# barathanaslan/whisper-ipa

Measured on AMD Instinct MI355X. Metric: audio-seconds/sec transcribed (whisper-small, 30s clips), higher is better.
Workload: dtype bf16

## Files before the change

whisper_ipa_amd/csrc/cross_absorbed.hip:

```cpp
#include <cstdlib>
#include <mutex>
#include <type_traits>

#include "attn_stream.h"
#include "wipa_common.h"

namespace {

constexpr int FT = 32;
constexpr long long XA_RESIDENT_MB_SHARED = 16;
constexpr long long XA_RESIDENT_MB_LONE = -1;
typedef __attribute__((address_space(3))) void* lds_ptr_a;
typedef int v2i32 __attribute__((ext_vector_type(2)));

struct AbsParams {
    const __bf16* qp;
    const __bf16* xa;
    float* part_m;
    float* part_l;
    float* part_o;
    int Tk, n_splits, tiles_per_split, H;
    int resident_groups;
};

constexpr int POLICY_DEFAULT = 0, POLICY_NT = 2;

__device__ __forceinline__ int swz(int row) { return (row & 7) << 1; }

// ... 207 lines not shown
typedef __bf16 bf16x4v __attribute__((ext_vector_type(4)));

template <int D, int NW_>
struct AbsCfg2 {
    static constexpr int NWV = NW_;
    static constexpr int GF = 16;
    static constexpr int ROWB = D * 2;
    static constexpr int SLOT = GF * ROWB;
    static constexpr int SMEM_LOOP = NWV * 2 * SLOT;
    static constexpr int MROW = D + 4;
    static constexpr int SMEM_MERGE = NWV * 16 * MROW * 4 + NWV * 32 * 4;
    static constexpr int SMEM = SMEM_LOOP > SMEM_MERGE ? SMEM_LOOP : SMEM_MERGE;
};

#define WIPA_TR8(X, A, IMM)                                                                                                          \
    asm volatile("ds_read_b64_tr_b16 %0, %8 offset:" #IMM "\n\tds_read_b64_tr_b16 %1, %9 offset:" #IMM                              \
                 "\n\tds_read_b64_tr_b16 %2, %10 offset:" #IMM "\n\tds_read_b64_tr_b16 %3, %11 offset:" #IMM                          \
                 "\n\tds_read_b64_tr_b16 %4, %12 offset:" #IMM "\n\tds_read_b64_tr_b16 %5, %13 offset:" #IMM                          \
                 "\n\tds_read_b64_tr_b16 %6, %14 offset:" #IMM "\n\tds_read_b64_tr_b16 %7, %15 offset:" #IMM "\n\ts_waitcnt lgkmcnt(0)" \
                 : "=&v"(X[0]), "=&v"(X[1]), "=&v"(X[2]), "=&v"(X[3]), "=&v"(X[4]), "=&v"(X[5]), "=&v"(X[6]), "=&v"(X[7])           \
                 : "v"(A[0]), "v"(A[1]), "v"(A[2]), "v"(A[3]), "v"(A[4]), "v"(A[5]), "v"(A[6]), "v"(A[7])                           \
                 : "memory")

template <int D, int NW_>
__global__ __launch_bounds__(64 * NW_, 1) void cross_absorbed_v2_kernel(AbsParams p) {
    typedef AbsCfg2<D, NW_> X;
    constexpr int NWV = X::NWV, GF = X::GF, ROWB = X::ROWB, SLOT = X::SLOT;
    constexpr int NDMA = SLOT / 1024;
    constexpr int KS = D / 32;
    constexpr int CT = D / 16;
    static_assert(SLOT % 1024 == 0 && NDMA <= 32 && CT % 8 == 0 && KS % 4 == 0 && CT / 8 <= 8 && D % 128 == 0, "width");
    extern __shared__ __attribute__((aligned(1024))) char smem[];
    const int tid = threadIdx.x, lane = tid & 63;
    const int wave = __builtin_amdgcn_readfirstlane(tid >> 6);
    const int l15 = lane & 15, g = lane >> 4;
    const int split = blockIdx.x, b = blockIdx.y;
    const int groups_total = (p.Tk + GF - 1) / GF;
    const int gps = 2 * p.tiles_per_split;
    const int g0 = split * gps;
    const int ng = max(0, min(gps, groups_total - g0));
    const int my_n = ng > wave ? (ng - wave + NWV - 1) / NWV : 0;
    const __bf16* xb = p.xa + (int64_t)b * p.Tk * D;
    char* my = smem + wave * (2 * SLOT);

    bf16x8 qf[KS];
    {
        const __bf16* qr = p.qp + ((int64_t)b * 16 + l15) * D + 8 * g;
// ... 60 lines not shown
            else if constexpr (NDMA == 16) asm volatile("s_waitcnt vmcnt(16)" ::: "memory");
            else if constexpr (NDMA == 12) asm volatile("s_waitcnt vmcnt(12)" ::: "memory");
            else asm volatile("s_waitcnt vmcnt(0)" ::: "memory");
        } else {
            asm volatile("s_waitcnt vmcnt(0)" ::: "memory");
        }
    };
    auto scores = [&](int slot, int i_local, float& mx) -> f32x4 {
        f32x4 s4[4] = {f32x4{0.f, 0.f, 0.f, 0.f}, f32x4{0.f, 0.f, 0.f, 0.f}, f32x4{0.f, 0.f, 0.f, 0.f}, f32x4{0.f, 0.f, 0.f, 0.f}};
        const int so = slot * SLOT;
#pragma unroll
        for (int ks = 0; ks < KS; ++ks) {
            const bf16x8 a = *reinterpret_cast<const bf16x8*>(sb[ks & 3] + so + 256 * (ks >> 2));
            s4[ks & 3] = __builtin_amdgcn_mfma_f32_16x16x32_bf16(a, qf[ks], s4[ks & 3], 0, 0, 0);
        }
        f32x4 s = (s4[0] + s4[1]) + (s4[2] + s4[3]);
        const int f0 = (g0 + wave + NWV * i_local) * GF;
        mx = NEG_BIG;
#pragma unroll
        for (int r = 0; r < 4; ++r) {
            if (f0 + 4 * g + r >= p.Tk) s[r] = NEG_BIG;
            mx = fmaxf(mx, s[r]);
        }
        mx = fmaxf(mx, __shfl_xor(mx, 16, 64));
        mx = fmaxf(mx, __shfl_xor(mx, 32, 64));
        return s;
    };
    constexpr float DRIFT = 40.f;
    f32x4 acc[CT];
    float m_ref = NEG_BIG, l_run = 0.f;
    bool exact = false;
    for (;;) {
#pragma unroll
        for (int c = 0; c < CT; ++c) acc[c] = f32x4{0.f, 0.f, 0.f, 0.f};
        l_run = 0.f;
        bool drifted = false;
        if (my_n > 0) stage(0, 0);
        if (my_n > 1) stage(1, 1);
        for (int i = 0; i < my_n; ++i) {
            const int slot = i & 1;
            wait_slot(i + 1 < my_n);
            float mx;
            const f32x4 s = scores(slot, i, mx);
            if (i == 0 && !exact) m_ref = mx;
            if (__builtin_amdgcn_ballot_w64(mx > m_ref + DRIFT) != 0) {
                drifted = true;
                break;
            }
            float ls = 0.f;
            bf16x4v pf;
#pragma unroll
            for (int r = 0; r < 4; ++r) {
                const float e = (s[r] <= NEG_TEST) ? 0.f : __expf(s[r] - m_ref);
                pf[r] = (__bf16)e;
                ls += e;
            }
            ls += __shfl_xor(ls, 16, 64);
            ls += __shfl_xor(ls, 32, 64);
            l_run += ls;
            {
                unsigned tas[8];
#pragma unroll
                for (int cc = 0; cc < 8; ++cc) tas[cc] = ta[cc] + slot * SLOT;
#define WIPA_PV_BLK(BLK, IMM)                                                                                                       \
    if constexpr (CT / 8 > BLK) {                                                                                                   \
        v2i32 x[8];                                                                                                                 \
        WIPA_TR8(x, tas, IMM);                                                                                                      \
        _Pragma("unroll") for (int cc = 0; cc < 8; ++cc) acc[8 * BLK + cc] =                                                       \
            __builtin_amdgcn_mfma_f32_16x16x16bf16_1k(pf, __builtin_bit_cast(bf16x4v, x[cc]), acc[8 * BLK + cc], 0, 0, 0);         \
    }
                WIPA_PV_BLK(0, 0)
                WIPA_PV_BLK(1, 256)
                WIPA_PV_BLK(2, 512)
                WIPA_PV_BLK(3, 768)
                WIPA_PV_BLK(4, 1024)
                WIPA_PV_BLK(5, 1280)
                WIPA_PV_BLK(6, 1536)
                WIPA_PV_BLK(7, 1792)
#undef WIPA_PV_BLK
            }
            asm volatile("" ::: "memory");
            if (i + 2 < my_n) stage(i + 2, slot);
        }
        if (!drifted) break;
        asm volatile("s_waitcnt vmcnt(0)" ::: "memory");
        float mt = NEG_BIG;
// ... 15 lines not shown
    asm volatile("s_waitcnt vmcnt(0)" ::: "memory");
    __syncthreads();
    constexpr int RS = X::MROW;
    float* so = reinterpret_cast<float*>(smem);
    float* sm = so + NWV * 16 * RS;
#pragma unroll
    for (int c = 0; c < CT; ++c)
#pragma unroll
        for (int r = 0; r < 4; ++r) so[(wave * 16 + 4 * g + r) * RS + 16 * c + l15] = acc[c][r];
    if (g == 0) {
        sm[wave * 16 + l15] = m_run;
        sm[NWV * 16 + wave * 16 + l15] = l_run;
    }
    __syncthreads();
    const int64_t ps = (int64_t)b * p.n_splits + split;
    float* po = p.part_o + ps * 16 * D;
    for (int hd = 0; hd < p.H; ++hd) {
        float mv[NWV], M = NEG_BIG;
#pragma unroll
        for (int v = 0; v < NWV; ++v) {
            mv[v] = sm[v * 16 + hd];
            M = fmaxf(M, mv[v]);
        }
        for (int c4 = tid; 4 * c4 < D; c4 += NWV * 64) {
            f32x4 o = {0.f, 0.f, 0.f, 0.f};
#pragma unroll
            for (int v = 0; v < NWV; ++v)
                o += __expf(mv[v] - M) * *reinterpret_cast<const f32x4*>(so + (v * 16 + hd) * RS + 4 * c4);
            *reinterpret_cast<f32x4*>(po + hd * D + 4 * c4) = o;
        }
    }
    if (tid < 16) {
        float M = NEG_BIG, Lsum = 0.f;
#pragma unroll
        for (int v = 0; v < NWV; ++v) M = fmaxf(M, sm[v * 16 + tid]);
#pragma unroll
        for (int v = 0; v < NWV; ++v) Lsum += __expf(sm[v * 16 + tid] - M) * sm[NWV * 16 + v * 16 + tid];
        p.part_m[ps * 16 + tid] = M;
        p.part_l[ps * 16 + tid] = Lsum;
    }
}
#undef WIPA_TR8

template <int D>
__global__ __launch_bounds__(64) void cross_absorb_q_kernel(const __bf16* __restrict__ q, int64_t q_rs, const __bf16* __restrict__ wkT,
                                                            __bf16* __restrict__ qp, int B, int H, float scale) {
    constexpr int CT = D / 4 / 16;
    const int lane = threadIdx.x & 63, wave = blockIdx.z;
    const int l15 = lane & 15, g = lane >> 4;
    const int h = blockIdx.x, b0 = blockIdx.y * 16;
    if (h >= H) {
        for (int e = lane; e < 16 * (D / 4); e += 64) {
            const int bb = b0 + e / (D / 4);
            if (bb < B) qp[((int64_t)bb * 16 + h) * D + wave * (D / 4) + e % (D / 4)] = (__bf16)0.f;
        }
        return;
    }
    const int bq = min(b0 + l15, B - 1);
    bf16x8 qa[2];
#pragma unroll
    for (int ks = 0; ks < 2; ++ks) qa[ks] = *reinterpret_cast<const bf16x8*>(q + (int64_t)bq * q_rs + h * 64 + 32 * ks + 8 * g);
    bf16x8 wb[CT][2];
#pragma unroll
    for (int i = 0; i < CT; ++i)
#pragma unroll
// ... 7 lines not shown
        for (int ks = 0; ks < 2; ++ks) acc = __builtin_amdgcn_mfma_f32_16x16x32_bf16(qa[ks], wb[i][ks], acc, 0, 0, 0);
#pragma unroll
        for (int r = 0; r < 4; ++r) {
            const int bb = b0 + 4 * g + r;
            if (bb < B) qp[((int64_t)bb * 16 + h) * D + c0 + l15] = (__bf16)(acc[r] * scale);
        }
    }
}

template <int D>
struct MergeCfg {
#ifndef WIPA_MERGE_KQ
#define WIPA_MERGE_KQ 96
#endif
#ifndef WIPA_MERGE_CL
#define WIPA_MERGE_CL 4
#endif
    static constexpr int KQ = (D % 96 == 0) ? WIPA_MERGE_KQ : (D == 512 ? 64 : 128);
    static constexpr int NWM = D / KQ;
    static constexpr int KS = KQ / 32;
    static constexpr int CL = WIPA_MERGE_CL;
};

template <int D, bool OUTP = false>
__global__ __launch_bounds__(64 * MergeCfg<D>::NWM) void cross_merge_proj_kernel(
    const float* __restrict__ part_m, const float* __restrict__ part_l, const float* __restrict__ part_o, int n_splits,
    const __bf16* __restrict__ wv, const float* __restrict__ bv, __bf16* __restrict__ out, int64_t o_rs, int B,
    const __bf16* __restrict__ wo = nullptr, const float* __restrict__ bo = nullptr, float* __restrict__ slabs_out = nullptr,
    int64_t slab_stride = 0) {
    constexpr int KQ = MergeCfg<D>::KQ, KS = MergeCfg<D>::KS, NWM = MergeCfg<D>::NWM;
    static_assert(KQ % 32 == 0 && NWM * KQ == D, "width");
    constexpr int CL = MergeCfg<D>::CL;
    constexpr int NTO = D / 16;
    constexpr int NTOW = (NTO + NWM - 1) / NWM;
    __shared__ __attribute__((aligned(16))) float red[NWM][CL][64 + 4];
    __shared__ __attribute__((aligned(16))) __bf16 vh[OUTP ? CL : 1][64 + 8];
    const int tid = threadIdx.x, lane = tid & 63, w = tid >> 6;
    const int l15 = lane & 15, g = lane >> 4;
    const int h = blockIdx.x, b0 = blockIdx.y * CL;
    const int bc = min(b0 + (l15 & (CL - 1)), B - 1);
    bf16x8 wq[4][KS];
#pragma unroll
    for (int nt = 0; nt < 4; ++nt)
#pragma unroll
        for (int ks = 0; ks < KS; ++ks)
            wq[nt][ks] = *reinterpret_cast<const bf16x8*>(wv + (int64_t)(h * 64 + 16 * nt + l15) * D + w * KQ + 32 * ks + 8 * g);
    bf16x8 wof[OUTP ? NTOW : 1][2];
    if constexpr (OUTP) {
#pragma unroll
        for (int i = 0; i < NTOW; ++i) {
            const int nt = min(w * NTOW + i, NTO - 1);
#pragma unroll
            for (int ks = 0; ks < 2; ++ks)
                wof[i][ks] = *reinterpret_cast<const bf16x8*>(wo + (int64_t)(16 * nt + l15) * D + h * 64 + 32 * ks + 8 * g);
        }
    }
    float pm[4], pl[4];
#pragma unroll
    for (int s = 0; s < 4; ++s) {
        const int sc = min(s, n_splits - 1);
        pm[s] = part_m[((int64_t)bc * n_splits + sc) * 16 + h];
        pl[s] = part_l[((int64_t)bc * n_splits + sc) * 16 + h];
    }
    f32x4 po[KS][4][2];
#pragma unroll
    for (int ks = 0; ks < KS; ++ks)
#pragma unroll
        for (int s = 0; s < 4; ++s) {
            const int sc = min(s, n_splits - 1);
            const float* pr = part_o + (((int64_t)bc * n_splits + sc) * 16 + h) * D + w * KQ + 32 * ks + 8 * g;
            po[ks][s][0] = *reinterpret_cast<const f32x4*>(pr);
            po[ks][s][1] = *reinterpret_cast<const f32x4*>(pr + 4);
        }
    __builtin_amdgcn_sched_barrier(0);
    float ws[4];
    {
        float M = NEG_BIG;
#pragma unroll
        for (int s = 0; s < 4; ++s)
            if (s < n_splits) M = fmaxf(M, pm[s]);
        float Lsum = 0.f;
#pragma unroll
        for (int s = 0; s < 4; ++s) {
            ws[s] = s < n_splits ? __expf(pm[s] - M) : 0.f;
            Lsum += ws[s] * pl[s];
        }
        const float inv = 1.0f / Lsum;
#pragma unroll
        for (int s = 0; s < 4; ++s) ws[s] *= inv;
    }
    f32x4 acc[4] = {f32x4{0.f, 0.f, 0.f, 0.f}, f32x4{0.f, 0.f, 0.f, 0.f}, f32x4{0.f, 0.f, 0.f, 0.f}, f32x4{0.f, 0.f, 0.f, 0.f}};
#pragma unroll
    for (int ks = 0; ks < KS; ++ks) {
        f32x4 lo = {0.f, 0.f, 0.f, 0.f}, hi = {0.f, 0.f, 0.f, 0.f};
#pragma unroll
        for (int s = 0; s < 4; ++s) {
            lo += ws[s] * po[ks][s][0];
            hi += ws[s] * po[ks][s][1];
        }
        bf16x8 a;
#pragma unroll
        for (int e = 0; e < 4; ++e) {
            a[e] = (__bf16)lo[e];
            a[4 + e] = (__bf16)hi[e];
        }
#pragma unroll
        for (int nt = 0; nt < 4; ++nt) acc[nt] = __builtin_amdgcn_mfma_f32_16x16x32_bf16(a, wq[nt][ks], acc[nt], 0, 0, 0);
    }
    if (4 * g < CL) {
#pragma unroll
        for (int nt = 0; nt < 4; ++nt)
#pragma unroll
            for (int r = 0; r < 4; ++r)
                if (4 * g + r < CL) red[w][4 * g + r][16 * nt + l15] = acc[nt][r];
    }
    __syncthreads();
    for (int e = tid; e < CL * 64; e += 64 * NWM) {
        const int row = e >> 6, j = e & 63;
        float o = 0.f;
#pragma unroll
        for (int v = 0; v < NWM; ++v) o += red[v][row][j];
// ... 156 lines not shown
        for (int e = tid; e < (16 - CG) * 64; e += 512) qh[CG + (e >> 6)][e & 63] = (__bf16)0.f;
    }
    __syncthreads();
    {
        const bf16x8 a0 = *reinterpret_cast<const bf16x8*>(&qh[l15][8 * g]);
        const bf16x8 a1 = *reinterpret_cast<const bf16x8*>(&qh[l15][32 + 8 * g]);
#pragma unroll
        for (int i = 0; i < NTW; ++i) {
            const int nt = wave * NTW + i;
            if (nt < NT) {
                f32x4 acc = {0.f, 0.f, 0.f, 0.f};
                acc = __builtin_amdgcn_mfma_f32_16x16x32_bf16(a0, wkf[i][0], acc, 0, 0, 0);
                acc = __builtin_amdgcn_mfma_f32_16x16x32_bf16(a1, wkf[i][1], acc, 0, 0, 0);
#pragma unroll
                for (int r = 0; r < 4; ++r) {
                    const int bb_ = b0 + 4 * g + r;
                    if (4 * g + r < CG && bb_ < p.B) p.qp[((int64_t)bb_ * 16 + h) * D + 16 * nt + l15] = (__bf16)(acc[r] * p.k_scale);
                }
            }
        }
    }
}

template <int D>
int launch_attn(const AbsParams& p_in, int B, hipStream_t s) {
    const char* e = getenv("WIPA_ABS_KERNEL");
    AbsParams p = p_in;
    p.resident_groups = wipa_cross_absorbed_resident_groups(B, D, p.Tk, p.n_splits);
    if ((e && atoi(e) == 1) || (D > 768 && !(e && atoi(e) == 2)))
        hipLaunchKernelGGL((cross_absorbed_kernel<D>), dim3(p.n_splits, B), dim3(64 * AbsCfg<D>::NW), AbsCfg<D>::SMEM, s, p);
    else if constexpr (D > 768)
        hipLaunchKernelGGL((cross_absorbed_v2_kernel<D, 2>), dim3(p.n_splits, B), dim3(128), (AbsCfg2<D, 2>::SMEM), s, p);
    else {
        static const int waves = [] { const char* w = getenv("WIPA_ABS_WAVES"); return w ? atoi(w) : 3; }();
        if (waves == 2) hipLaunchKernelGGL((cross_absorbed_v2_kernel<D, 2>), dim3(p.n_splits, B), dim3(128), (AbsCfg2<D, 2>::SMEM), s, p);
        else hipLaunchKernelGGL((cross_absorbed_v2_kernel<D, 3>), dim3(p.n_splits, B), dim3(192), (AbsCfg2<D, 3>::SMEM), s, p);
    }
    return WIPA_OK;
}

AbsParams abs_params(void* scratch, int B, int d, int Tk, int S, int H, const void* xa) {
    char* sc = (char*)scratch;
    AbsParams p = {};
    p.qp = (const __bf16*)sc; p.xa = (const __bf16*)xa;
    p.part_m = (float*)(sc + (size_t)B * 16 * d * 2);
    p.part_l = p.part_m + (size_t)B * S * 16;
    p.part_o = p.part_l + (size_t)B * S * 16;
    p.Tk = Tk; p.n_splits = S; p.H = H;
    const int tiles = (Tk + FT - 1) / FT;
    p.tiles_per_split = (tiles + S - 1) / S;
    return p;
}

template <typename F>
int for_width(int d, F f) {
    if (d == 384) return f(std::integral_constant<int, 384>());
    if (d == 512) return f(std::integral_constant<int, 512>());
    if (d == 768) return f(std::integral_constant<int, 768>());
    if (d == 1024) return f(std::integral_constant<int, 1024>());
// ... 27 lines not shown
    if (mb == INT64_MIN) mb = (S <= 2) ? XA_RESIDENT_MB_SHARED : XA_RESIDENT_MB_LONE;
    return wipa_cross_absorbed_resident_groups_for(B, d, Tk, S, mb < 0 ? -1 : mb * 1000000);
}

extern "C" size_t wipa_cross_absorbed_scratch_bytes(int B, int d, int Tk) {
    (void)Tk;
    return (size_t)B * 16 * d * 2 + (size_t)B * 4 * 16 * (2 + (size_t)d) * 4 + 1024;
}

extern "C" int wipa_cross_absorbed_init(int d) {
    static std::mutex mu;
    static bool done[4] = {false, false, false, false};
    const int wi = d == 384 ? 0 : d == 512 ? 1 : d == 768 ? 2 : d == 1024 ? 3 : -1;
    if (wi < 0) return WIPA_ERR_ARG;
    std::lock_guard<std::mutex> lk(mu);
    if (done[wi]) return WIPA_OK;
    hipError_t e = hipSuccess;
    for_width(d, [&](auto width) {
        constexpr int D = decltype(width)::value;
        e = hipFuncSetAttribute(reinterpret_cast<const void*>(&cross_absorbed_kernel<D>), hipFuncAttributeMaxDynamicSharedMemorySize,
                                AbsCfg<D>::SMEM);
        if constexpr (D <= 768) {
            if (e == hipSuccess)
                e = hipFuncSetAttribute(reinterpret_cast<const void*>(&cross_absorbed_v2_kernel<D, 3>),
                                        hipFuncAttributeMaxDynamicSharedMemorySize, AbsCfg2<D, 3>::SMEM);
        }
        if (e == hipSuccess)
            e = hipFuncSetAttribute(reinterpret_cast<const void*>(&cross_absorbed_v2_kernel<D, 2>),
                                    hipFuncAttributeMaxDynamicSharedMemorySize, AbsCfg2<D, 2>::SMEM);
        return WIPA_OK;
    });
    WIPA_CHECK_HIP(e);
    done[wi] = true;
    return WIPA_OK;
}

extern "C" int wipa_cross_absorbed_stream(const void* xa, void* scratch, size_t scratch_bytes, int B, int H, int d, int Tk, int n_splits,
                                          wipa_stream_t stream) {
    WIPA_REQUIRE(xa && scratch && B > 0 && H >= 1 && H <= 16 && d == H * 64 && (d == 384 || d == 512 || d == 768 || d == 1024) && Tk >= 1 &&
                     n_splits >= 0 && n_splits <= 4,
                 "wipa_cross_absorbed_stream: bad arguments");
    WIPA_REQUIRE(scratch_bytes >= wipa_cross_absorbed_scratch_bytes(B, d, Tk), "wipa_cross_absorbed_stream: scratch too small");
    const int rc0 = wipa_cross_absorbed_init(d);
    if (rc0 != WIPA_OK) return rc0;
    const int S = wipa_cross_absorbed_splits(n_splits, Tk);
    const AbsParams p = abs_params(scratch, B, d, Tk, S, H, xa);
    const int rc = for_width(d, [&](auto width) { return launch_attn<decltype(width)::value>(p, B, (hipStream_t)stream); });
    if (rc != WIPA_OK) return rc;
    WIPA_LAUNCH_CHECK();
    return WIPA_OK;
}

extern "C" int wipa_cross_absorbed_attention(const void* q, int64_t q_row_stride, const void* wkT, const void* xa, const void* wv,
                                             const float* bv, void* out, int64_t out_row_stride, void* scratch, size_t scratch_bytes,
                                             int B, int H, int d, int Tk, float k_scale, int n_splits, wipa_stream_t stream) {
    WIPA_REQUIRE(q && wkT && xa && wv && bv && out && scratch, "wipa_cross_absorbed_attention: null pointer");
    WIPA_REQUIRE(n_splits >= 0 && n_splits <= 4, "wipa_cross_absorbed_attention: n_splits %d (0 = default, 1..4)", n_splits);
    WIPA_REQUIRE(B > 0 && B <= 65535 && H >= 1 && H <= 16 && d == H * 64 && (d == 384 || d == 512 || d == 768 || d == 1024) && Tk >= 1,
                 "wipa_cross_absorbed_attention: bf16, <= 16 heads of 64, d in {384, 512, 768, 1024} (got H=%d d=%d)", H, d);
    WIPA_REQUIRE(q_row_stride % 8 == 0 && out_row_stride >= d && ((uintptr_t)q % 16) == 0 && ((uintptr_t)xa % 16) == 0 &&
                     ((uintptr_t)wkT % 16) == 0 && ((uintptr_t)wv % 16) == 0 && ((uintptr_t)scratch % 16) == 0,
                 "wipa_cross_absorbed_attention: operands must be 16-byte aligned");
    WIPA_REQUIRE((int64_t)Tk * d * 2 < ((int64_t)1 << 31), "wipa_cross_absorbed_attention: clip too long for 32-bit tile offsets");
    WIPA_REQUIRE(scratch_bytes >= wipa_cross_absorbed_scratch_bytes(B, d, Tk), "wipa_cross_absorbed_attention: scratch too small");
    hipStream_t s = (hipStream_t)stream;
    {
        const int rc0 = wipa_cross_absorbed_init(d);
        if (rc0 != WIPA_OK) return rc0;
    }
    const int S = wipa_cross_absorbed_splits(n_splits, Tk);
    const AbsParams p = abs_params(scratch, B, d, Tk, S, H, xa);
    const dim3 gq(16, (B + 15) / 16, 4), gm(H, (B + WIPA_MERGE_CL - 1) / WIPA_MERGE_CL);
    const char* st_env = getenv("WIPA_ABS_STAGES");
    const int stages = st_env ? atoi(st_env) : 7;
    const int rc = for_width(d, [&](auto width) {
        constexpr int D = decltype(width)::value;
        int rc = WIPA_OK;
        if (stages & 1)
            hipLaunchKernelGGL((cross_absorb_q_kernel<D>), gq, dim3(64), 0, s, (const __bf16*)q, q_row_stride, (const __bf16*)wkT,
                               const_cast<__bf16*>(p.qp), B, H, k_scale);
        if (stages & 2) rc = launch_attn<D>(p, B, s);
        if (rc == WIPA_OK && (stages & 4))
            hipLaunchKernelGGL((cross_merge_proj_kernel<D>), gm, dim3(64 * MergeCfg<D>::NWM), 0, s, p.part_m, p.part_l, p.part_o, S,
                               (const __bf16*)wv, bv, (__bf16*)out, out_row_stride, B);
        return rc;
    });
    if (rc != WIPA_OK) return rc;
    WIPA_LAUNCH_CHECK();
    return WIPA_OK;
}

static int absorbed_block(const wipa_cross_block_desc* c, const void* wkT, const void* wv, const float* bv, const void* wo, const float* bo,
                          float* slabs_out, int64_t slab_stride, void* scratch, size_t scratch_bytes, wipa_stream_t stream);

extern "C" int wipa_decode_cross_absorbed_block(const wipa_cross_block_desc* c, const void* wkT, const void* wv, const float* bv, void* scratch,
                                                size_t scratch_bytes, wipa_stream_t stream) {
    WIPA_REQUIRE(c && c->out, "wipa_decode_cross_absorbed_block: null pointer");
    return absorbed_block(c, wkT, wv, bv, nullptr, nullptr, nullptr, 0, scratch, scratch_bytes, stream);
}

extern "C" int wipa_decode_cross_absorbed_block_out(const wipa_cross_block_desc* c, const void* wkT, const void* wv, const float* bv,
                                                    const void* wo, const float* bo, float* slabs_out, int64_t slab_stride, void* scratch,
                                                    size_t scratch_bytes, wipa_stream_t stream) {
    WIPA_REQUIRE(c && wo && bo && slabs_out && slab_stride >= (int64_t)c->B * c->d && ((uintptr_t)wo % 16) == 0,
                 "wipa_decode_cross_absorbed_block_out: null pointer / short slab stride");
    return absorbed_block(c, wkT, wv, bv, wo, bo, slabs_out, slab_stride, scratch, scratch_bytes, stream);
}

static int absorbed_block(const wipa_cross_block_desc* c, const void* wkT, const void* wv, const float* bv, const void* wo, const float* bo,
                          float* slabs_out, int64_t slab_stride, void* scratch, size_t scratch_bytes, wipa_stream_t stream) {
    WIPA_REQUIRE(c && c->x_in && c->x_out && c->ln_w && c->ln_b && c->wq && c->bq && c->kv && (c->out || wo) && wkT && wv && bv && scratch,
                 "wipa_decode_cross_absorbed_block: null pointer");
    WIPA_REQUIRE(c->x_in != c->x_out, "wipa_decode_cross_absorbed_block: x_out must not alias x_in");
    const int B = c->B, H = c->H, d = c->d, Tk = c->Tk;
    WIPA_REQUIRE(c->dtype == WIPA_BF16 && B > 0 && B <= 65535 * 16 && H >= 1 && H <= 16 && d == H * 64 &&
                     (d == 384 || d == 512 || d == 768 || d == 1024) && Tk >= 1 && c->n_slabs >= 0 && c->n_slabs <= 4 && !c->bias_o &&
                     c->cross_splits >= 0 && c->cross_splits <= 4,
                 "wipa_decode_cross_absorbed_block: bf16, <= 16 heads of 64, d in {384, 512, 768, 1024}, <= 4 slabs, no separate bias, "
                 "cross_splits 0..4");
    WIPA_REQUIRE(c->n_slabs == 0 || c->slabs, "wipa_decode_cross_absorbed_block: slabs missing");
    WIPA_REQUIRE((int64_t)Tk * d * 2 < ((int64_t)1 << 31), "wipa_decode_cross_absorbed_block: clip too long for 32-bit tile offsets");
    WIPA_REQUIRE(scratch_bytes >= wipa_cross_absorbed_scratch_bytes(B, d, Tk), "wipa_decode_cross_absorbed_block: scratch too small");
    hipStream_t s = (hipStream_t)stream;
    const int S = wipa_cross_absorbed_splits(c->cross_splits, Tk);
    const AbsParams p = abs_params(scratch, B, d, Tk, S, H, c->kv);
    AbsPrologueParams q = {};
    q.x_in = c->x_in; q.x_out = c->x_out; q.slabs = c->slabs; q.ln_w = c->ln_w; q.ln_b = c->ln_b;
    q.wq = (const __bf16*)c->wq; q.bq = c->bq; q.wkT = (const __bf16*)wkT; q.qp = const_cast<__bf16*>(p.qp);
    q.slab_stride = c->slab_stride; q.n_slabs = c->n_slabs; q.B = B; q.H = H;
    q.eps = c->eps; q.q_scale = c->qk_scale; q.k_scale = c->qk_scale;
    static const int cg = [] { const char* e = getenv("WIPA_ABS_PROLOGUE_CLIPS"); return e ? atoi(e) : 8; }();
    const dim3 gp(H, cg == 8 ? (B + 7) / 8 : (B + 15) / 16), gm(H, (B + WIPA_MERGE_CL - 1) / WIPA_MERGE_CL);
    const int rc = for_width(d, [&](auto width) {
        constexpr int D = decltype(width)::value;
        if (cg == 8) hipLaunchKernelGGL((cross_absorb_prologue_kernel<D, 8>), gp, dim3(512), 0, s, q);
        else hipLaunchKernelGGL((cross_absorb_prologue_kernel<D, 16>), gp, dim3(512), 0, s, q);
        const int rc = launch_attn<D>(p, B, s);
        if (rc == WIPA_OK && wo)
            hipLaunchKernelGGL((cross_merge_proj_kernel<D, true>), gm, dim3(64 * MergeCfg<D>::NWM), 0, s, p.part_m, p.part_l, p.part_o, S,
                               (const __bf16*)wv, bv, (__bf16*)nullptr, (int64_t)d, B, (const __bf16*)wo, bo, slabs_out, slab_stride);
        else if (rc == WIPA_OK)
            hipLaunchKernelGGL((cross_merge_proj_kernel<D>), gm, dim3(64 * MergeCfg<D>::NWM), 0, s, p.part_m, p.part_l, p.part_o, S,
                               (const __bf16*)wv, bv, (__bf16*)c->out, (int64_t)d, B);
        return rc;
    });
    if (rc != WIPA_OK) return rc;
    WIPA_LAUNCH_CHECK();
    return WIPA_OK;
}
```

whisper_ipa_amd/csrc/runtime.hip:

```cpp
#include <algorithm>
#include <cstdarg>
#include <cstdlib>
#include <cstring>
#include <strings.h>
#include <map>
#include <mutex>
#include <tuple>
#include <vector>

#include "wipa_common.h"

static thread_local char g_err[512] = "";
void wipa_set_error(const char* fmt, ...) {
    va_list ap;
    va_start(ap, fmt);
    vsnprintf(g_err, sizeof(g_err), fmt, ap);
    va_end(ap);
}
extern "C" const char* wipa_last_error(void) { return g_err; }
extern "C" int wipa_version(void) { return 100; }

extern "C" int wipa_stream_create_cu_limited(int n_cus, wipa_stream_t* out) {
    int dev = 0, total = 0;
    WIPA_CHECK_HIP(hipGetDevice(&dev));
// ... 862 lines not shown
    RulesScope rules_scope(rules);
    W8Scope w8_scope(cfg, w);
    const wipa_dec_layout L = dec_layout(cfg, B);
    RT_CALL(state_fits("wipa_decoder_run", L, state_bytes));
    char* st = (char*)state;
    hipStream_t s = (hipStream_t)stream;
    RT_CALL(init_before_capture(cfg));
    if (n_steps == 0) return WIPA_OK;
    WIPA_CHECK_HIP(hipMemsetAsync(done_counter_of(st, L), 0, sizeof(int32_t), s));
    if (step_needs_head(cfg, B)) RT_CALL(enqueue_step_head(cfg, w, st, L, B, stream));
    const bool lean_ok = !use_fused_step(cfg, B) && logits_fused(cfg, B);
    struct LeanScope {
        explicit LeanScope(bool v) { t_lean_logits = v; }
        ~LeanScope() { t_lean_logits = false; }
    };
    if (!use_graph || !graphs_allowed()) {
        for (int i = 0; i < n_steps; ++i) {
            LeanScope lean(lean_ok && i + 1 < n_steps);
            RT_CALL(enqueue_decode_step(cfg, w, st, L, B, n_init, eot, mask_first, mask_always, stream));
        }
        return WIPA_OK;
    }
    WIPA_REQUIRE(s != nullptr, "wipa_decoder_run: graph capture needs a non-default stream");
    const int variant = cfg->dtype * 2 + t_f32_split + 4 * decode_mode(cfg, B) + 16 * cfg->dec_w_dtype + 64 * cfg->dec_cross_absorbed * (absorbed_block_fused() ? 2 : 1) + 256 * (int)tail_fused() + 512 * (int)absorbed_merge_out() + 1024 * cfg->dec_cross_splits + 8192 * (int)lean_ok;
    auto step_graph = [&](bool lean, hipGraphExec_t* out) -> int {
        hipGraphExec_t exec = nullptr;
        const GraphKey key(state, (const void*)w, (const void*)mask_first, (const void*)mask_always, B, n_init, eot, variant, cfg->weights_generation,
                           lean ? 2 : 0, rules ? rules->timestamp_begin : 0, rules ? rules->no_timestamps : 0,
                           rules ? rules->max_initial_timestamp_index : 0);
        {
            std::lock_guard<std::mutex> lk(g_graph_mu);
            auto it = g_graphs.find(key);
            if (it != g_graphs.end()) exec = it->second;
        }
        if (!exec) {
            hipGraph_t graph = nullptr;
            WIPA_CHECK_HIP(hipStreamBeginCapture(s, hipStreamCaptureModeRelaxed));
            int rc;
            {
                LeanScope scope(lean);
                rc = enqueue_decode_step(cfg, w, st, L, B, n_init, eot, mask_first, mask_always, stream);
            }
            const hipError_t ee = hipStreamEndCapture(s, &graph);
            if (rc != WIPA_OK) {
                if (graph) hipGraphDestroy(graph);
                return rc;
            }
// ... 24 lines not shown
                                          const wipa_decode_rules* rules, wipa_stream_t stream) {
    RT_CALL(cfg_check(cfg));
    SplitScope split_scope(cfg);
    WIPA_REQUIRE(w && state && mask_first && mask_always && B > 0, "wipa_decoder_prefill: bad arguments");
    RT_CALL(rules_servable("wipa_decoder_prefill_rules", cfg, B, eot, rules));
    RulesScope rules_scope(rules);
    WIPA_REQUIRE(n_init >= 1 && n_init <= MAX_PROMPT, "wipa_decoder_prefill: 1..%d prompt tokens (got %d)", MAX_PROMPT, n_init);
    W8Scope w8_scope(cfg, w);
    const wipa_dec_layout L = dec_layout(cfg, B);
    RT_CALL(state_fits("wipa_decoder_prefill", L, state_bytes));
    char* st = (char*)state;
    auto enqueue = [&]() -> int {
        if (n_init == 1) {
            if (step_needs_head(cfg, B)) RT_CALL(enqueue_step_head(cfg, w, st, L, B, stream));
            return enqueue_decode_step(cfg, w, st, L, B, n_init, eot, mask_first, mask_always, stream);
        }
        return enqueue_prefill(cfg, w, st, L, B, n_init, eot, mask_first, mask_always, stream);
    };
    hipStream_t s = (hipStream_t)stream;
    RT_CALL(init_before_capture(cfg));
    WIPA_CHECK_HIP(hipMemsetAsync(done_counter_of(st, L), 0, sizeof(int32_t), s));
    if (!use_graph || s == nullptr || !graphs_allowed()) return enqueue();
    hipGraphExec_t exec = nullptr;
    const GraphKey key(state, (const void*)w, (const void*)mask_first, (const void*)mask_always, B, n_init, eot, cfg->dtype * 2 + t_f32_split + 4 * decode_mode(cfg, B) + 16 * cfg->dec_w_dtype + 64 * cfg->dec_cross_absorbed * (absorbed_block_fused() ? 2 : 1) + 256 * (int)tail_fused() + 512 * (int)absorbed_merge_out() + 1024 * cfg->dec_cross_splits + 8192 * (int)(!use_fused_step(cfg, B) && logits_fused(cfg, B)), cfg->weights_generation, 1,
                       rules ? rules->timestamp_begin : 0, rules ? rules->no_timestamps : 0, rules ? rules->max_initial_timestamp_index : 0);
    {
        std::lock_guard<std::mutex> lk(g_graph_mu);
        auto it = g_graphs.find(key);
        if (it != g_graphs.end()) exec = it->second;
    }
    if (!exec) {
        hipGraph_t graph = nullptr;
        WIPA_CHECK_HIP(hipStreamBeginCapture(s, hipStreamCaptureModeRelaxed));
        const int rc = enqueue();
        const hipError_t ee = hipStreamEndCapture(s, &graph);
        if (rc != WIPA_OK) {
            if (graph) hipGraphDestroy(graph);
            return rc;
        }
        WIPA_CHECK_HIP(ee);
        WIPA_CHECK_HIP(hipGraphInstantiate(&exec, graph, nullptr, nullptr, 0));
        WIPA_CHECK_HIP(hipGraphDestroy(graph));
        std::lock_guard<std::mutex> lk(g_graph_mu);
        g_graphs[key] = exec;
    }
    WIPA_CHECK_HIP(hipGraphLaunch(exec, s));
    return WIPA_OK;
// ... 119 lines not shown
```

whisper_ipa_amd/csrc/wipa_common.h:

```cpp
#pragma once
#include <hip/hip_runtime.h>
#include <stdint.h>
#include <stdio.h>

#include "wipa.h"

typedef __attribute__((ext_vector_type(8))) __bf16 bf16x8;
typedef __attribute__((ext_vector_type(4))) __bf16 bf16x4;
typedef __attribute__((ext_vector_type(4))) float f32x4;
typedef __attribute__((ext_vector_type(16))) float f32x16;

#define WIPA_WAVE 64

void wipa_set_error(const char* fmt, ...);
int wipa_decode_fused_init();
int wipa_gemm_init();

#define WIPA_CHECK_HIP(expr)                                                        \
    do {                                                                            \
        hipError_t _e = (expr);                                                     \
        if (_e != hipSuccess) {                                                     \
            wipa_set_error("%s:%d %s -> %s", __FILE__, __LINE__, #expr, hipGetErrorString(_e)); \
            return WIPA_ERR_HIP;                                                    \
        }                                                                           \
    } while (0)

#define WIPA_REQUIRE(cond, ...)                \
    do {                                       \
        if (!(cond)) {                         \
            wipa_set_error(__VA_ARGS__);       \
            return WIPA_ERR_ARG;               \
        }                                      \
    } while (0)

#define WIPA_LAUNCH_CHECK()                                                          \
    do {                                                                             \
        hipError_t _e = hipGetLastError();                                           \
        if (_e != hipSuccess) {                                                      \
            wipa_set_error("%s:%d launch -> %s", __FILE__, __LINE__, hipGetErrorString(_e)); \
// ... 123 lines not shown
```

Before: 26860.

## Pipeline LDS transpose reads with PV MFMAs and specialize merge by split count

Adds a pipelined variant of the cross-attention absorbed kernel that issues the next block's ds_read_b64_tr_b16 transposed LDS reads before running the current block's MFMAs, using partial lgkmcnt waits instead of a full wait per block. Wave reductions now use permlane16/32 swaps instead of shuffles. The merge kernel is templated on the split count, which drops the clamping and predication, and its per-wave exp weights are hoisted out of the inner loop. An env-selected loop variant (default 1) enables both changes and is folded into the graph cache key; the cost is more register pressure and more template instantiations.

```diff
diff --git a/whisper_ipa_amd/csrc/cross_absorbed.hip b/whisper_ipa_amd/csrc/cross_absorbed.hip
--- a/whisper_ipa_amd/csrc/cross_absorbed.hip
+++ b/whisper_ipa_amd/csrc/cross_absorbed.hip
@@ -4,6 +4,12 @@
 
 #include "attn_stream.h"
 #include "wipa_common.h"
+
+int wipa_cross_absorbed_loop_variant() {
+    const char* e = getenv("WIPA_ABS_LOOP");
+    const int v = e ? atoi(e) : 1;
+    return (v >= 0 && v <= 3) ? v : 1;
+}
 
 namespace {
 
@@ -257,7 +263,47 @@
                  : "v"(A[0]), "v"(A[1]), "v"(A[2]), "v"(A[3]), "v"(A[4]), "v"(A[5]), "v"(A[6]), "v"(A[7])                           \
                  : "memory")
 
-template <int D, int NW_>
+#define WIPA_TR8_ISSUE(Y, A, IMM)                                                                                                    \
+    asm volatile("ds_read_b64_tr_b16 %0, %8 offset:" #IMM "\n\tds_read_b64_tr_b16 %1, %9 offset:" #IMM                              \
+                 "\n\tds_read_b64_tr_b16 %2, %10 offset:" #IMM "\n\tds_read_b64_tr_b16 %3, %11 offset:" #IMM                          \
+                 "\n\tds_read_b64_tr_b16 %4, %12 offset:" #IMM "\n\tds_read_b64_tr_b16 %5, %13 offset:" #IMM                          \
+                 "\n\tds_read_b64_tr_b16 %6, %14 offset:" #IMM "\n\tds_read_b64_tr_b16 %7, %15 offset:" #IMM                          \
+                 : "=&v"(Y[0]), "=&v"(Y[1]), "=&v"(Y[2]), "=&v"(Y[3]), "=&v"(Y[4]), "=&v"(Y[5]), "=&v"(Y[6]), "=&v"(Y[7])           \
+                 : "v"(A[0]), "v"(A[1]), "v"(A[2]), "v"(A[3]), "v"(A[4]), "v"(A[5]), "v"(A[6]), "v"(A[7])                           \
+                 : "memory")
+#define WIPA_TR8_NEXT(Y, X, A, IMM)                                                                                                  \
+    asm volatile("ds_read_b64_tr_b16 %0, %16 offset:" #IMM "\n\tds_read_b64_tr_b16 %1, %17 offset:" #IMM                            \
+                 "\n\tds_read_b64_tr_b16 %2, %18 offset:" #IMM "\n\tds_read_b64_tr_b16 %3, %19 offset:" #IMM                          \
+                 "\n\tds_read_b64_tr_b16 %4, %20 offset:" #IMM "\n\tds_read_b64_tr_b16 %5, %21 offset:" #IMM                          \
+                 "\n\tds_read_b64_tr_b16 %6, %22 offset:" #IMM "\n\tds_read_b64_tr_b16 %7, %23 offset:" #IMM "\n\ts_waitcnt lgkmcnt(8)" \
+                 : "=&v"(Y[0]), "=&v"(Y[1]), "=&v"(Y[2]), "=&v"(Y[3]), "=&v"(Y[4]), "=&v"(Y[5]), "=&v"(Y[6]), "=&v"(Y[7]),          \
+                   "+v"(X[0]), "+v"(X[1]), "+v"(X[2]), "+v"(X[3]), "+v"(X[4]), "+v"(X[5]), "+v"(X[6]), "+v"(X[7])                   \
+                 : "v"(A[0]), "v"(A[1]), "v"(A[2]), "v"(A[3]), "v"(A[4]), "v"(A[5]), "v"(A[6]), "v"(A[7])                           \
+                 : "memory")
+#define WIPA_TR8_LAST(X)                                                                                                             \
+    asm volatile("s_waitcnt lgkmcnt(0)"                                                                                              \
+                 : "+v"(X[0]), "+v"(X[1]), "+v"(X[2]), "+v"(X[3]), "+v"(X[4]), "+v"(X[5]), "+v"(X[6]), "+v"(X[7])                   \
+                 :                                                                                                                   \
+                 : "memory")
+
+__device__ __forceinline__ float max_xor16(float v) {
+    const auto r = __builtin_amdgcn_permlane16_swap(__float_as_uint(v), __float_as_uint(v), false, false);
+    return fmaxf(__uint_as_float(r[0]), __uint_as_float(r[1]));
+}
+__device__ __forceinline__ float max_xor32(float v) {
+    const auto r = __builtin_amdgcn_permlane32_swap(__float_as_uint(v), __float_as_uint(v), false, false);
+    return fmaxf(__uint_as_float(r[0]), __uint_as_float(r[1]));
+}
+__device__ __forceinline__ float sum_xor16(float v) {
+    const auto r = __builtin_amdgcn_permlane16_swap(__float_as_uint(v), __float_as_uint(v), false, false);
+    return __uint_as_float(r[0]) + __uint_as_float(r[1]);
+}
+__device__ __forceinline__ float sum_xor32(float v) {
+    const auto r = __builtin_amdgcn_permlane32_swap(__float_as_uint(v), __float_as_uint(v), false, false);
+    return __uint_as_float(r[0]) + __uint_as_float(r[1]);
+}
+
+template <int D, int NW_, bool PIPE>
 __global__ __launch_bounds__(64 * NW_, 1) void cross_absorbed_v2_kernel(AbsParams p) {
     typedef AbsCfg2<D, NW_> X;
     constexpr int NWV = X::NWV, GF = X::GF, ROWB = X::ROWB, SLOT = X::SLOT;
@@ -364,8 +410,13 @@
             if (f0 + 4 * g + r >= p.Tk) s[r] = NEG_BIG;
             mx = fmaxf(mx, s[r]);
         }
-        mx = fmaxf(mx, __shfl_xor(mx, 16, 64));
-        mx = fmaxf(mx, __shfl_xor(mx, 32, 64));
+        if constexpr (PIPE) {
+            mx = max_xor16(mx);
+            mx = max_xor32(mx);
+        } else {
+            mx = fmaxf(mx, __shfl_xor(mx, 16, 64));
+            mx = fmaxf(mx, __shfl_xor(mx, 32, 64));
+        }
         return s;
     };
     constexpr float DRIFT = 40.f;
@@ -389,6 +440,14 @@
                 drifted = true;
                 break;
             }
+            unsigned tas[8];
+#pragma unroll
+            for (int cc = 0; cc < 8; ++cc) tas[cc] = ta[cc] + slot * SLOT;
+            v2i32 xe[8], xo[8];
+            if constexpr (PIPE) {
+                WIPA_TR8_ISSUE(xe, tas, 0);
+                __builtin_amdgcn_sched_barrier(0);
+            }
             float ls = 0.f;
             bf16x4v pf;
 #pragma unroll
@@ -397,13 +456,37 @@
                 pf[r] = (__bf16)e;
                 ls += e;
             }
-            ls += __shfl_xor(ls, 16, 64);
-            ls += __shfl_xor(ls, 32, 64);
-            l_run += ls;
-            {
-                unsigned tas[8];
-#pragma unroll
-                for (int cc = 0; cc < 8; ++cc) tas[cc] = ta[cc] + slot * SLOT;
+            if constexpr (!PIPE) {
+                ls += __shfl_xor(ls, 16, 64);
+                ls += __shfl_xor(ls, 32, 64);
+                l_run += ls;
+            }
+            if constexpr (PIPE) {
+                constexpr int NB = CT / 8;
+                __builtin_amdgcn_sched_barrier(0);
+#define WIPA_PV_STEP(BLK, CUR, NXT, IMM_NEXT)                                                                                       \
+    if constexpr (NB > BLK) {                                                                                                       \
+        if constexpr (NB > BLK + 1) WIPA_TR8_NEXT(NXT, CUR, tas, IMM_NEXT);                                                         \
+        else {                                                                                                                      \
+            __builtin_amdgcn_sched_barrier(0);                       \
+            WIPA_TR8_LAST(CUR);                                                                                                     \
+        }                                                                                                                           \
+        _Pragma("unroll") for (int cc = 0; cc < 8; ++cc) acc[8 * BLK + cc] =                                                       \
+            __builtin_amdgcn_mfma_f32_16x16x16bf16_1k(pf, __builtin_bit_cast(bf16x4v, CUR[cc]), acc[8 * BLK + cc], 0, 0, 0);       \
+    }
+                WIPA_PV_STEP(0, xe, xo, 256)
+                WIPA_PV_STEP(1, xo, xe, 512)
+                WIPA_PV_STEP(2, xe, xo, 768)
+                WIPA_PV_STEP(3, xo, xe, 1024)
+                WIPA_PV_STEP(4, xe, xo, 1280)
+                WIPA_PV_STEP(5, xo, xe, 1536)
+                WIPA_PV_STEP(6, xe, xo, 1792)
+                WIPA_PV_STEP(7, xo, xe, 2048)
+#undef WIPA_PV_STEP
+                ls = sum_xor16(ls);
+                ls = sum_xor32(ls);
+                l_run += ls;
+            } else {
 #define WIPA_PV_BLK(BLK, IMM)                                                                                                       \
     if constexpr (CT / 8 > BLK) {                                                                                                   \
         v2i32 x[8];                                                                                                                 \
@@ -465,11 +548,14 @@
             mv[v] = sm[v * 16 + hd];
             M = fmaxf(M, mv[v]);
         }
+        float wgt[NWV];
+#pragma unroll
+        for (int v = 0; v < NWV; ++v) wgt[v] = __expf(mv[v] - M);
         for (int c4 = tid; 4 * c4 < D; c4 += NWV * 64) {
             f32x4 o = {0.f, 0.f, 0.f, 0.f};
 #pragma unroll
             for (int v = 0; v < NWV; ++v)
-                o += __expf(mv[v] - M) * *reinterpret_cast<const f32x4*>(so + (v * 16 + hd) * RS + 4 * c4);
+                o += wgt[v] * *reinterpret_cast<const f32x4*>(so + (v * 16 + hd) * RS + 4 * c4);
             *reinterpret_cast<f32x4*>(po + hd * D + 4 * c4) = o;
         }
     }
@@ -484,6 +570,9 @@
     }
 }
 #undef WIPA_TR8
+#undef WIPA_TR8_ISSUE
+#undef WIPA_TR8_NEXT
+#undef WIPA_TR8_LAST
 
 template <int D>
 __global__ __launch_bounds__(64) void cross_absorb_q_kernel(const __bf16* __restrict__ q, int64_t q_rs, const __bf16* __restrict__ wkT,
@@ -537,7 +626,7 @@
     static constexpr int CL = WIPA_MERGE_CL;
 };
 
-template <int D, bool OUTP = false>
+template <int D, bool OUTP = false, int NS = 4>
 __global__ __launch_bounds__(64 * MergeCfg<D>::NWM) void cross_merge_proj_kernel(
     const float* __restrict__ part_m, const float* __restrict__ part_l, const float* __restrict__ part_o, int n_splits,
     const __bf16* __restrict__ wv, const float* __restrict__ bv, __bf16* __restrict__ out, int64_t o_rs, int B,
@@ -570,48 +659,49 @@
                 wof[i][ks] = *reinterpret_cast<const bf16x8*>(wo + (int64_t)(16 * nt + l15) * D + h * 64 + 32 * ks + 8 * g);
         }
     }
-    float pm[4], pl[4];
-#pragma unroll
-    for (int s = 0; s < 4; ++s) {
-        const int sc = min(s, n_splits - 1);
+    float pm[NS], pl[NS];
+#pragma unroll
+    for (int s = 0; s < NS; ++s) {
+        const int sc = NS == 4 ? min(s, n_splits - 1) : s;
         pm[s] = part_m[((int64_t)bc * n_splits + sc) * 16 + h];
         pl[s] = part_l[((int64_t)bc * n_splits + sc) * 16 + h];
     }
-    f32x4 po[KS][4][2];
+    f32x4 po[KS][NS][2];
 #pragma unroll
     for (int ks = 0; ks < KS; ++ks)
 #pragma unroll
-        for (int s = 0; s < 4; ++s) {
-            const int sc = min(s, n_splits - 1);
+        for (int s = 0; s < NS; ++s) {
+            const int sc = NS == 4 ? min(s, n_splits - 1) : s;
             const float* pr = part_o + (((int64_t)bc * n_splits + sc) * 16 + h) * D + w * KQ + 32 * ks + 8 * g;
             po[ks][s][0] = *reinterpret_cast<const f32x4*>(pr);
             po[ks][s][1] = *reinterpret_cast<const f32x4*>(pr + 4);
         }
     __builtin_amdgcn_sched_barrier(0);
-    float ws[4];
+    float ws[NS];
     {
         float M = NEG_BIG;
 #pragma unroll
-        for (int s = 0; s < 4; ++s)
-            if (s < n_splits) M = fmaxf(M, pm[s]);
+        for (int s = 0; s < NS; ++s)
+            if (NS < 4 || s < n_splits) M = fmaxf(M, pm[s]);
         float Lsum = 0.f;
 #pragma unroll
-        for (int s = 0; s < 4; ++s) {
-            ws[s] = s < n_splits ? __expf(pm[s] - M) : 0.f;
-            Lsum += ws[s] * pl[s];
+        for (int s = 0; s < NS; ++s) {
+            ws[s] = (NS < 4 || s < n_splits) ? __expf(pm[s] - M) : 0.f;
+            Lsum = __builtin_fmaf(ws[s], pl[s], Lsum);
         }
         const float inv = 1.0f / Lsum;
 #pragma unroll
-        for (int s = 0; s < 4; ++s) ws[s] *= inv;
+        for (int s = 0; s < NS; ++s) ws[s] *= inv;
     }
     f32x4 acc[4] = {f32x4{0.f, 0.f, 0.f, 0.f}, f32x4{0.f, 0.f, 0.f, 0.f}, f32x4{0.f, 0.f, 0.f, 0.f}, f32x4{0.f, 0.f, 0.f, 0.f}};
 #pragma unroll
     for (int ks = 0; ks < KS; ++ks) {
         f32x4 lo = {0.f, 0.f, 0.f, 0.f}, hi = {0.f, 0.f, 0.f, 0.f};
 #pragma unroll
-        for (int s = 0; s < 4; ++s) {
-            lo += ws[s] * po[ks][s][0];
-            hi += ws[s] * po[ks][s][1];
+        for (int s = 0; s < NS; ++s) {
+            const f32x4 w4 = {ws[s], ws[s], ws[s], ws[s]};
+            lo = __builtin_elementwise_fma(w4, po[ks][s][0], lo);
+            hi = __builtin_elementwise_fma(w4, po[ks][s][1], hi);
         }
         bf16x8 a;
 #pragma unroll
@@ -814,19 +904,33 @@
     }
 }
 
+template <int D, bool OUTP, typename... Args>
+void launch_merge(int lv, int S, dim3 grid, hipStream_t s, Args... args) {
+    constexpr int T = 64 * MergeCfg<D>::NWM;
+    const int ns = (lv == 1 || lv == 3) ? S : 4;
+    if (ns == 1) hipLaunchKernelGGL((cross_merge_proj_kernel<D, OUTP, 1>), grid, dim3(T), 0, s, args...);
+    else if (ns == 2) hipLaunchKernelGGL((cross_merge_proj_kernel<D, OUTP, 2>), grid, dim3(T), 0, s, args...);
+    else if (ns == 3) hipLaunchKernelGGL((cross_merge_proj_kernel<D, OUTP, 3>), grid, dim3(T), 0, s, args...);
+    else hipLaunchKernelGGL((cross_merge_proj_kernel<D, OUTP, 4>), grid, dim3(T), 0, s, args...);
+}
+
 template <int D>
-int launch_attn(const AbsParams& p_in, int B, hipStream_t s) {
+int launch_attn(int lv, const AbsParams& p_in, int B, hipStream_t s) {
     const char* e = getenv("WIPA_ABS_KERNEL");
+    const bool pipe = lv == 1 || lv == 2;
     AbsParams p = p_in;
     p.resident_groups = wipa_cross_absorbed_resident_groups(B, D, p.Tk, p.n_splits);
     if ((e && atoi(e) == 1) || (D > 768 && !(e && atoi(e) == 2)))
         hipLaunchKernelGGL((cross_absorbed_kernel<D>), dim3(p.n_splits, B), dim3(64 * AbsCfg<D>::NW), AbsCfg<D>::SMEM, s, p);
-    else if constexpr (D > 768)
-        hipLaunchKernelGGL((cross_absorbed_v2_kernel<D, 2>), dim3(p.n_splits, B), dim3(128), (AbsCfg2<D, 2>::SMEM), s, p);
-    else {
+    else if constexpr (D > 768) {
+        if (pipe) hipLaunchKernelGGL((cross_absorbed_v2_kernel<D, 2, true>), dim3(p.n_splits, B), dim3(128), (AbsCfg2<D, 2>::SMEM), s, p);
+        else hipLaunchKernelGGL((cross_absorbed_v2_kernel<D, 2, false>), dim3(p.n_splits, B), dim3(128), (AbsCfg2<D, 2>::SMEM), s, p);
+    } else {
         static const int waves = [] { const char* w = getenv("WIPA_ABS_WAVES"); return w ? atoi(w) : 3; }();
-        if (waves == 2) hipLaunchKernelGGL((cross_absorbed_v2_kernel<D, 2>), dim3(p.n_splits, B), dim3(128), (AbsCfg2<D, 2>::SMEM), s, p);
-        else hipLaunchKernelGGL((cross_absorbed_v2_kernel<D, 3>), dim3(p.n_splits, B), dim3(192), (AbsCfg2<D, 3>::SMEM), s, p);
+        if (waves == 2 && pipe) hipLaunchKernelGGL((cross_absorbed_v2_kernel<D, 2, true>), dim3(p.n_splits, B), dim3(128), (AbsCfg2<D, 2>::SMEM), s, p);
+        else if (waves == 2) hipLaunchKernelGGL((cross_absorbed_v2_kernel<D, 2, false>), dim3(p.n_splits, B), dim3(128), (AbsCfg2<D, 2>::SMEM), s, p);
+        else if (pipe) hipLaunchKernelGGL((cross_absorbed_v2_kernel<D, 3, true>), dim3(p.n_splits, B), dim3(192), (AbsCfg2<D, 3>::SMEM), s, p);
+        else hipLaunchKernelGGL((cross_absorbed_v2_kernel<D, 3, false>), dim3(p.n_splits, B), dim3(192), (AbsCfg2<D, 3>::SMEM), s, p);
     }
     return WIPA_OK;
 }
@@ -900,11 +1004,17 @@
                                 AbsCfg<D>::SMEM);
         if constexpr (D <= 768) {
             if (e == hipSuccess)
-                e = hipFuncSetAttribute(reinterpret_cast<const void*>(&cross_absorbed_v2_kernel<D, 3>),
+                e = hipFuncSetAttribute(reinterpret_cast<const void*>(&cross_absorbed_v2_kernel<D, 3, true>),
                                         hipFuncAttributeMaxDynamicSharedMemorySize, AbsCfg2<D, 3>::SMEM);
+            if (e == hipSuccess)
+                e = hipFuncSetAttribute(reinterpret_cast<const void*>(&cross_absorbed_v2_kernel<D, 3, false>),
+                                        hipFuncAttributeMaxDynamicSharedMemorySize, AbsCfg2<D, 3>::SMEM);
         }
         if (e == hipSuccess)
-            e = hipFuncSetAttribute(reinterpret_cast<const void*>(&cross_absorbed_v2_kernel<D, 2>),
+            e = hipFuncSetAttribute(reinterpret_cast<const void*>(&cross_absorbed_v2_kernel<D, 2, true>),
+                                    hipFuncAttributeMaxDynamicSharedMemorySize, AbsCfg2<D, 2>::SMEM);
+        if (e == hipSuccess)
+            e = hipFuncSetAttribute(reinterpret_cast<const void*>(&cross_absorbed_v2_kernel<D, 2, false>),
                                     hipFuncAttributeMaxDynamicSharedMemorySize, AbsCfg2<D, 2>::SMEM);
         return WIPA_OK;
     });
@@ -923,7 +1033,7 @@
     if (rc0 != WIPA_OK) return rc0;
     const int S = wipa_cross_absorbed_splits(n_splits, Tk);
     const AbsParams p = abs_params(scratch, B, d, Tk, S, H, xa);
-    const int rc = for_width(d, [&](auto width) { return launch_attn<decltype(width)::value>(p, B, (hipStream_t)stream); });
+    const int rc = for_width(d, [&](auto width) { return launch_attn<decltype(width)::value>(wipa_cross_absorbed_loop_variant(), p, B, (hipStream_t)stream); });
     if (rc != WIPA_OK) return rc;
     WIPA_LAUNCH_CHECK();
     return WIPA_OK;
@@ -949,6 +1059,7 @@
     const int S = wipa_cross_absorbed_splits(n_splits, Tk);
     const AbsParams p = abs_params(scratch, B, d, Tk, S, H, xa);
     const dim3 gq(16, (B + 15) / 16, 4), gm(H, (B + WIPA_MERGE_CL - 1) / WIPA_MERGE_CL);
+    const int lv = wipa_cross_absorbed_loop_variant();
     const char* st_env = getenv("WIPA_ABS_STAGES");
     const int stages = st_env ? atoi(st_env) : 7;
     const int rc = for_width(d, [&](auto width) {
@@ -957,10 +1068,10 @@
         if (stages & 1)
             hipLaunchKernelGGL((cross_absorb_q_kernel<D>), gq, dim3(64), 0, s, (const __bf16*)q, q_row_stride, (const __bf16*)wkT,
                                const_cast<__bf16*>(p.qp), B, H, k_scale);
-        if (stages & 2) rc = launch_attn<D>(p, B, s);
+        if (stages & 2) rc = launch_attn<D>(lv, p, B, s);
         if (rc == WIPA_OK && (stages & 4))
-            hipLaunchKernelGGL((cross_merge_proj_kernel<D>), gm, dim3(64 * MergeCfg<D>::NWM), 0, s, p.part_m, p.part_l, p.part_o, S,
-                               (const __bf16*)wv, bv, (__bf16*)out, out_row_stride, B);
+            launch_merge<D, false>(lv, S, gm, s, (const float*)p.part_m, (const float*)p.part_l, (const float*)p.part_o, S, (const __bf16*)wv, bv,
+                                   (__bf16*)out, out_row_stride, B, (const __bf16*)nullptr, (const float*)nullptr, (float*)nullptr, (int64_t)0);
         return rc;
     });
     if (rc != WIPA_OK) return rc;
@@ -1007,19 +1118,20 @@
     q.wq = (const __bf16*)c->wq; q.bq = c->bq; q.wkT = (const __bf16*)wkT; q.qp = const_cast<__bf16*>(p.qp);
     q.slab_stride = c->slab_stride; q.n_slabs = c->n_slabs; q.B = B; q.H = H;
     q.eps = c->eps; q.q_scale = c->qk_scale; q.k_scale = c->qk_scale;
+    const int lv = wipa_cross_absorbed_loop_variant();
     static const int cg = [] { const char* e = getenv("WIPA_ABS_PROLOGUE_CLIPS"); return e ? atoi(e) : 8; }();
     const dim3 gp(H, cg == 8 ? (B + 7) / 8 : (B + 15) / 16), gm(H, (B + WIPA_MERGE_CL - 1) / WIPA_MERGE_CL);
     const int rc = for_width(d, [&](auto width) {
         constexpr int D = decltype(width)::value;
         if (cg == 8) hipLaunchKernelGGL((cross_absorb_prologue_kernel<D, 8>), gp, dim3(512), 0, s, q);
         else hipLaunchKernelGGL((cross_absorb_prologue_kernel<D, 16>), gp, dim3(512), 0, s, q);
-        const int rc = launch_attn<D>(p, B, s);
+        const int rc = launch_attn<D>(lv, p, B, s);
         if (rc == WIPA_OK && wo)
-            hipLaunchKernelGGL((cross_merge_proj_kernel<D, true>), gm, dim3(64 * MergeCfg<D>::NWM), 0, s, p.part_m, p.part_l, p.part_o, S,
-                               (const __bf16*)wv, bv, (__bf16*)nullptr, (int64_t)d, B, (const __bf16*)wo, bo, slabs_out, slab_stride);
+            launch_merge<D, true>(lv, S, gm, s, (const float*)p.part_m, (const float*)p.part_l, (const float*)p.part_o, S, (const __bf16*)wv, bv,
+                                  (__bf16*)nullptr, (int64_t)d, B, (const __bf16*)wo, bo, slabs_out, slab_stride);
         else if (rc == WIPA_OK)
-            hipLaunchKernelGGL((cross_merge_proj_kernel<D>), gm, dim3(64 * MergeCfg<D>::NWM), 0, s, p.part_m, p.part_l, p.part_o, S,
-                               (const __bf16*)wv, bv, (__bf16*)c->out, (int64_t)d, B);
+            launch_merge<D, false>(lv, S, gm, s, (const float*)p.part_m, (const float*)p.part_l, (const float*)p.part_o, S, (const __bf16*)wv, bv,
+                                   (__bf16*)c->out, (int64_t)d, B, (const __bf16*)nullptr, (const float*)nullptr, (float*)nullptr, (int64_t)0);
         return rc;
     });
     if (rc != WIPA_OK) return rc;
diff --git a/whisper_ipa_amd/csrc/runtime.hip b/whisper_ipa_amd/csrc/runtime.hip
--- a/whisper_ipa_amd/csrc/runtime.hip
+++ b/whisper_ipa_amd/csrc/runtime.hip
@@ -908,7 +908,7 @@
         return WIPA_OK;
     }
     WIPA_REQUIRE(s != nullptr, "wipa_decoder_run: graph capture needs a non-default stream");
-    const int variant = cfg->dtype * 2 + t_f32_split + 4 * decode_mode(cfg, B) + 16 * cfg->dec_w_dtype + 64 * cfg->dec_cross_absorbed * (absorbed_block_fused() ? 2 : 1) + 256 * (int)tail_fused() + 512 * (int)absorbed_merge_out() + 1024 * cfg->dec_cross_splits + 8192 * (int)lean_ok;
+    const int variant = cfg->dtype * 2 + t_f32_split + 4 * decode_mode(cfg, B) + 16 * cfg->dec_w_dtype + 64 * cfg->dec_cross_absorbed * (absorbed_block_fused() ? 2 : 1) + 256 * (int)tail_fused() + 512 * (int)absorbed_merge_out() + 1024 * cfg->dec_cross_splits + 8192 * (int)lean_ok + 16384 * (cfg->dec_cross_absorbed ? wipa_cross_absorbed_loop_variant() : 0);
     auto step_graph = [&](bool lean, hipGraphExec_t* out) -> int {
         hipGraphExec_t exec = nullptr;
         const GraphKey key(state, (const void*)w, (const void*)mask_first, (const void*)mask_always, B, n_init, eot, variant, cfg->weights_generation,
@@ -979,7 +979,7 @@
     WIPA_CHECK_HIP(hipMemsetAsync(done_counter_of(st, L), 0, sizeof(int32_t), s));
     if (!use_graph || s == nullptr || !graphs_allowed()) return enqueue();
     hipGraphExec_t exec = nullptr;
-    const GraphKey key(state, (const void*)w, (const void*)mask_first, (const void*)mask_always, B, n_init, eot, cfg->dtype * 2 + t_f32_split + 4 * decode_mode(cfg, B) + 16 * cfg->dec_w_dtype + 64 * cfg->dec_cross_absorbed * (absorbed_block_fused() ? 2 : 1) + 256 * (int)tail_fused() + 512 * (int)absorbed_merge_out() + 1024 * cfg->dec_cross_splits + 8192 * (int)(!use_fused_step(cfg, B) && logits_fused(cfg, B)), cfg->weights_generation, 1,
+    const GraphKey key(state, (const void*)w, (const void*)mask_first, (const void*)mask_always, B, n_init, eot, cfg->dtype * 2 + t_f32_split + 4 * decode_mode(cfg, B) + 16 * cfg->dec_w_dtype + 64 * cfg->dec_cross_absorbed * (absorbed_block_fused() ? 2 : 1) + 256 * (int)tail_fused() + 512 * (int)absorbed_merge_out() + 1024 * cfg->dec_cross_splits + 8192 * (int)(!use_fused_step(cfg, B) && logits_fused(cfg, B)) + 16384 * (cfg->dec_cross_absorbed ? wipa_cross_absorbed_loop_variant() : 0), cfg->weights_generation, 1,
                        rules ? rules->timestamp_begin : 0, rules ? rules->no_timestamps : 0, rules ? rules->max_initial_timestamp_index : 0);
     {
         std::lock_guard<std::mutex> lk(g_graph_mu);
diff --git a/whisper_ipa_amd/csrc/wipa_common.h b/whisper_ipa_amd/csrc/wipa_common.h
--- a/whisper_ipa_amd/csrc/wipa_common.h
+++ b/whisper_ipa_amd/csrc/wipa_common.h
@@ -15,6 +15,7 @@
 void wipa_set_error(const char* fmt, ...);
 int wipa_decode_fused_init();
 int wipa_gemm_init();
+int wipa_cross_absorbed_loop_variant();
 
 #define WIPA_CHECK_HIP(expr)                                                        \
     do {                                                                            \
```

Measured after the change: 27690 (median of 6 runs). 3.1% higher.
